# tavildar/Polar

Measured on AMD Instinct MI355X. Metric: codewords/s (N=2048 K=1024 L=32 LLR-SCL), higher is better.
Workload: dtype f64

## Files before the change

polar_amd/build.py:

```python
import os
import shutil
import subprocess
import sys

HERE = os.path.dirname(os.path.abspath(__file__))
ROOT = os.path.dirname(HERE)
CSRC = os.path.join(HERE, "csrc")
INC = os.path.join(ROOT, "include")
LIB = os.path.join(HERE, "libpolar_amd.so")
BUILD = os.path.join(HERE, "_build")
FLAGS_LIST32 = ["-mllvm", "-amdgpu-sched-strategy=max-memory-clause", "-mllvm", "-amdgpu-use-amdgpu-trackers"] + \
               os.environ.get("POLAR_LIST32_FLAGS", "").split()
FLAGS_LAT = os.environ.get("POLAR_LAT_FLAGS", "").split()
SOURCES = [("polar_kernels.hip", ["POLAR_ED_TU=0"], "", []), ("polar_kernels.hip", ["POLAR_ED_TU=1"], ".ed", []),
           ("polar_kernels.hip", ["POLAR_ED_TU=2"], ".ed32", FLAGS_LIST32), ("polar_kernels.hip", ["POLAR_ED_TU=3"], ".lat", FLAGS_LAT),
           ("polar_kernels.hip", ["POLAR_ED_TU=4"], ".list", []),
           ("polar_kernels_sc.hip", [], "", []), ("polar_kernels_p1.hip", [], "", []), ("polar_channel.hip", [], "", []),
           ("polar_construct.hip", [], "", []), ("polar_kernels_mlc.hip", [], "", []), ("polar_kernels_ga.hip", [], "", [])] + \
          [(f, [], "", []) for f in ("polar_handle.cpp", "polar_decode.cpp", "polar_hostpipe.cpp", "polar_montecarlo.cpp", "polar_multi.cpp",
                                     "polar_debug.cpp", "polar_ga.cpp", "polar_bicm.cpp", "polar_list.cpp", "polar_mlc.cpp")]
TEST_HOOK_SOURCES = ("polar_montecarlo.cpp", "polar_debug.cpp")
LIB_TEST = os.path.join(HERE, "libpolar_amd_test.so")
KNOWN_DEFS = {"POLAR_MARGIN", "POLAR_SLOTHIST", "SCLAT_PROF", "POLAR_DEV_GS32", "POLAR_DEV_ONE", "POLAR_NO_FIXED_N",
              "POLAR_NO_GUARD_INT", "POLAR_NO_COLD_HINTS", "OCC", "ED_NR"}
ARCH = os.environ.get("POLAR_ARCH", "gfx950")
_flags_ok = {}


def _probe_flags(flags):
    key = tuple(flags)
    if key not in _flags_ok:
# ... 179 lines not shown
```

polar_amd/csrc/polar_debug.cpp:

```cpp
#include "polar_multi.h"
#include "polar_amd_debug.h"

extern "C" {

int polar_debug_weak_leaves(const polar_code_t *h) { return polar_get_weak_leaves(h); }

int polar_debug_set(polar_code_t *h, const char *key, long value) {
    if (!h || !key) return fail(POLAR_E_ARG, "NULL argument");
    polar_code::Knobs &k = h->knobs;
    const std::string s(key);
    if (s == "mode_override") { if (value < -1 || value > 2) return fail(POLAR_E_ARG, "mode_override must be -1 (none), 0, 1 or 2"); k.mode_override = (int)value; }
    else if (s == "sc_no_fold") k.sc_no_fold = value != 0;
    else if (s == "no_tables") k.no_tables = value != 0;
    else if (s == "no_fuse_front") k.no_fuse_front = value != 0;
    else if (s == "no_prefix") h->prefix_on = (value == 0);
    else if (s == "no_rccl") { k.no_rccl = value != 0; multi_release(h, false); }
    else if (s == "force_rccl") { k.force_rccl = value != 0; multi_release(h, false); }
#ifdef POLAR_TEST_HOOKS
    else if (s == "host_fail_alloc") k.host_fail_alloc = value;
    else if (s == "share_device") { k.share_device = value != 0; multi_release(h, false); }
    else if (s == "fail_device") k.fail_device = (int)value;
    else if (s == "fail_collective") k.fail_collective = (int)value;
#endif
    else if (s == "lat_max_b") k.lat_max_b = value;
    else if (s == "list_chunk_cw") { if (value < 0) return fail(POLAR_E_ARG, "list_chunk_cw must be >= 0"); k.list_chunk_cw = value; }
    else if (s == "host_pipe_min_bytes") k.host_pipe_min_bytes = value;
    else if (s == "host_chunk_bytes") k.host_chunk_bytes = value;
    else if (s == "host_lanes") { if (value < 0 || value > HostPipe::kMaxLanes) return fail(POLAR_E_ARG, "host_lanes must be 0 (default) or 1 .. %d", HostPipe::kMaxLanes); k.host_lanes = value; }
// ... 15 lines not shown
long polar_debug_get(const polar_code_t *h, const char *key) {
    if (!key) return -1;
    const std::string s(key);
    if (s == "allocs") return (long)g_allocs.load();
    if (s == "comm_inits") return (long)polar_debug_comm_inits();
    if (!h) return -1;
    if (s == "test_hooks") {
#ifdef POLAR_TEST_HOOKS
        return 1;
#else
        return 0;
#endif
    }
    if (s == "weak_leaves") return h->weak_leaves;
    if (s == "mode_override") return h->knobs.mode_override;
    if (s == "last_rounds") return h->last_rounds;
    if (s == "last_round_max_per_device") return h->last_round_max_per_device;
    if (s == "worker_threads_started") return h->worker_threads_started;
    if (s.compare(0, 9, "round_us_") == 0) {
        if (h->round_us.empty()) return 0;
        std::vector<long> v(h->round_us);
        if (s == "round_us_count") return (long)v.size();
        if (s == "round_us_first") return v.front();
        std::sort(v.begin(), v.end());
        if (s == "round_us_min") return v.front();
        if (s == "round_us_max") return v.back();
        if (s == "round_us_median") return v[v.size() / 2];
        return -1;
    }
    if (s == "multi_poisoned") return h->multi_poisoned ? 1 : 0;
// ... 14 lines not shown
```

polar_amd/csrc/polar_decode.cpp:

```cpp
#include "polar_host.h"

namespace {

int effective_mode(const polar_code *h) { return h->knobs.mode_override >= 0 ? h->knobs.mode_override : h->mode; }
long lat_resident(const polar_code *h, int gs) {
    const size_t lds = polar_decode_lat_lds_bytes(h->N, gs, h->W);
    return lds <= h->lds_per_block ? (long)h->num_cu * std::min<long>(4, (long)(h->lds_per_block / lds)) : 0;
}
bool use_sc_lat(const polar_code *h, long B) {
    return h->n <= polar_sc_lat_max_log() && polar_sc_lat_lds_bytes(h->N, (int)h->sc_lat_ops.size()) <= h->lds_per_block &&
           h->knobs.lat_max_b >= 0 && B <= (h->knobs.lat_max_b ? h->knobs.lat_max_b : 2048);
}

struct Call {
    polar_code *h;
    const void *d_llr; int llr_fmt; long B; const unsigned int *n_dev; int L; uint8_t *d_out; double *d_pm;
    hipStream_t st; void *ev_start, *ev_stop; int phase; Deferred *deferred;
    BatchGeometry g; PolarDecodeParams p;
};

int batch_setup(polar_code *h, long B, int L, BatchGeometry &g) {
    if (!batch_geometry(h, B, L, true, g)) return fail(POLAR_E_ARG, "lds_log %d does not fit the LDS", g.lds_log);
    if ((size_t)g.grid * g.big * 64 + 64 > h->d_llr_scr.cap) {
        const size_t per_wave = g.big * 64 * sizeof(double) + 1;
// ... 80 lines not shown
    if (int rc = prefix_params(h, g.gs, p)) return rc;
    HIP_TRY(hipMemsetAsync(p.work, 0, sizeof(unsigned int), c.st));
    if (p.prefix_q) HIP_TRY(polar_launch_prefix(p, false, nullptr, c.st));
    if (c.ev_start) HIP_TRY(hipEventRecord((hipEvent_t)c.ev_start, c.st));
    HIP_TRY(polar_launch_decode_llr(p, g.gs, g.lds_log, g.pipe, g.grid, false, c.st));
    if (c.ev_stop) HIP_TRY(hipEventRecord((hipEvent_t)c.ev_stop, c.st));
    return POLAR_OK;
}

int decode_batch_ed(Call &c) {
    polar_code *h = c.h; const BatchGeometry &g = c.g;
    PolarDecodeParams &p = c.p;
    const long B = c.B;
    int rc;
    if ((rc = prefix_params(h, g.gs, p))) return rc;
    HIP_TRY(hipMemsetAsync(p.work, 0, sizeof(unsigned int), c.st));
    if ((rc = h->d_ech.ensure((size_t)B * h->N))) return rc;
    if ((rc = h->d_flags.ensure((size_t)B))) return rc;
    if ((rc = h->d_list.ensure((size_t)B))) return rc;
    if ((rc = h->d_count.ensure(1))) return rc;
    HIP_TRY(hipMemsetAsync(h->d_count.p, 0, sizeof(unsigned int), c.st));
    const bool fuse_front = p.prefix_q > 0 && polar_prefix_is_staged(h->N) && !h->knobs.no_fuse_front;
    if (!fuse_front) HIP_TRY(polar_launch_ed_front(c.d_llr, c.llr_fmt, h->d_ech.p, h->d_flags.p, h->d_tabs.p, h->N, B, c.n_dev, c.st));
    PolarDecodeParams pe = p;
    pe.llr = h->d_ech.p; pe.llr_fmt = POLAR_LLR_F64; pe.flags = h->d_flags.p;
    if (g.gs == 32 && !g.pipe && h->N >= 1024 && p.prefix_q > 0 && !h->knobs.no_tables) {
        if ((rc = h->d_tab_scr.ensure((size_t)g.grid * g.G * 3 * h->N + 64))) return rc;
        if ((rc = h->d_var_scr.ensure((size_t)g.grid * (h->N / 32) * 64 + 64))) return rc;
        pe.tab_scr = h->d_tab_scr.p; pe.var_scr = h->d_var_scr.p;
    }
    if (pe.prefix_q && fuse_front) {
        PolarDecodeParams pp = pe;
        pp.llr = (const double *)c.d_llr; pp.llr_fmt = c.llr_fmt;
        HIP_TRY(polar_launch_prefix(pp, true, h->d_ech.p, c.st));
    } else if (pe.prefix_q) HIP_TRY(polar_launch_prefix(pe, true, nullptr, c.st));
    if (c.ev_start) HIP_TRY(hipEventRecord((hipEvent_t)c.ev_start, c.st));
    HIP_TRY(polar_launch_decode_llr(pe, g.gs, g.lds_log, g.pipe, g.grid, true, c.st));
    if (c.ev_stop) HIP_TRY(hipEventRecord((hipEvent_t)c.ev_stop, c.st));
    HIP_TRY(polar_launch_ed_collect(h->d_flags.p, B, c.n_dev, h->d_list.p, h->d_count.p, c.st));
    return fallback_pass(p, g, h->d_list.p, h->d_count.p, nullptr, h->weak_leaves ? g.grid : 64 * g.wpb, c.st);
}

}

Family polar_host::choose_family(const polar_code *h, long B, int L, bool want_pm) {
    const int mode = effective_mode(h), gs = pow2ceil(L);
    if (L == 1 && mode != 1 && !want_pm) return use_sc_lat(h, B) ? Family::ScLat : Family::Sc8;
    const bool ed = gs >= 4 && mode != 1;
    const long resident = lat_resident(h, gs);
    if ((gs == 2 || (ed && (gs == 4 || gs == 8))) && h->knobs.lat_max_b >= 0 && resident > 0 &&
        B <= (h->knobs.lat_max_b ? h->knobs.lat_max_b : 2 * resident)) return Family::ListLat;
// ... 55 lines not shown
void polar_host::fill_enc(const polar_code *h, PolarEncodeParams &p) {
    memset(&p, 0, sizeof p);
    p.n = h->n; p.N = h->N; p.K = h->K; p.crc = h->crc;
    p.order = h->d_order.p; p.crcm = h->d_crcm.p;
    p.stride = 1;
    p.info_block_div = 100;
}

int polar_host::decode_impl(polar_code *h, const void *d_llr, int llr_fmt, long B, const unsigned int *n_dev, int L, uint8_t *d_out,
                            double *d_pm, void *stream, void *ev_start, void *ev_stop, int phase, Deferred *deferred) {
    if (deferred) *deferred = Deferred::None;
    int rc = check_args(h && d_llr && d_out, L, B);
    if (rc || B == 0) return rc;
    DevGuard dg_;
    if ((rc = ensure_device(h, dg_))) return rc;
    if ((rc = h->d_work.ensure(1))) return rc;
    const Family fam = choose_family(h, B, L, d_pm != nullptr);
    Call c{h, d_llr, llr_fmt, B, n_dev, L, d_out, d_pm, (hipStream_t)stream, ev_start, ev_stop, phase, deferred, {}, {}};
    if (!(fam == Family::ListLat && effective_mode(h) == 1) && (rc = batch_setup(h, B, L, c.g))) return rc;
    base_params(h, L, B, c.p);
    c.p.llr = (const double *)d_llr; c.p.llr_fmt = llr_fmt; c.p.out = d_out; c.p.pm_out = d_pm; c.p.n_dev = n_dev;
    switch (fam) {
        case Family::Sc8: case Family::ScLat: return decode_sc8(c, fam == Family::ScLat);
        case Family::ListLat: return decode_list_lat(c);
        case Family::BatchLlr: return decode_batch_llr(c);
        case Family::BatchEd: break;
    }
    return decode_batch_ed(c);
}

extern "C" {
// ... 127 lines not shown
    int rc = check_args(true, L, B);
    if (rc || B == 0) return rc;
    DevGuard dg_;
    if ((rc = ensure_device(h, dg_))) return rc;
    DevBuf<double> llr, pm;
    DevBuf<uint8_t> out;
    if ((rc = llr.ensure((size_t)B * h->N + 1)) || (rc = out.ensure((size_t)B * h->K)) || (rc = pm.ensure((size_t)B))) { llr.release(); out.release(); pm.release(); return rc; }
    rc = polar_synth_llr_dev(h, 1, 0, B, polar_snr_sqrt_linear(h, 2.0), llr.p, nullptr, nullptr);
    const int top = std::min(pow2ceil(L), POLAR_MAX_LIST);
    for (int l = 1; l <= top && !rc; l <<= 1) {
        rc = polar_decode_scl_llr_batch_dev(h, llr.p, B, l, out.p, nullptr, nullptr);
        if (!rc && l <= 8) rc = polar_decode_scl_llr_batch_dev(h, llr.p, 1, l, out.p, nullptr, nullptr);
        if (!rc && l == 1) rc = polar_decode_scl_llr_batch_dev(h, llr.p, B, l, out.p, pm.p, nullptr);
        if (!rc && l == 1) rc = polar_decode_scl_llr_batch_dev(h, llr.p + 1, B, l, out.p, nullptr, nullptr);
    }
    hipError_t e = hipDeviceSynchronize();
    llr.release(); out.release(); pm.release();
    if (!rc && e != hipSuccess) return fail(POLAR_E_DEVICE, "polar_reserve: %s", hipGetErrorString(e));
    return rc;
}

int polar_count_errors_dev(polar_code_t *h, const uint8_t *d_a, const uint8_t *d_b, long B,
                           unsigned long long *d_err_count, void *stream) {
    int rc = check_args(h && d_a && d_b && d_err_count, kNoList, B);
    if (rc || B == 0) return rc;
    DevGuard dg_;
    if ((rc = ensure_device(h, dg_))) return rc;
    HIP_TRY(polar_launch_count_errors(d_a, d_b, B, h->K, d_err_count, nullptr, (hipStream_t)stream));
    return POLAR_OK;
}
// ... 3 lines not shown
```

polar_amd/csrc/polar_edom.h:

```cpp
#pragma once
#include <hip/hip_runtime.h>
#include <stdint.h>

#include "polar_device.h"

#ifndef POLAR_NO_COLD_HINTS
#define POLAR_UNLIKELY(x) __builtin_expect(!!(x), 0)
#define POLAR_LIKELY(x) __builtin_expect(!!(x), 1)
#else
#define POLAR_UNLIKELY(x) (x)
#define POLAR_LIKELY(x) (x)
#endif
#define POLAR_UNLIKELY2(x) POLAR_UNLIKELY(x)
#define POLAR_LIKELY2(x) POLAR_LIKELY(x)

namespace {

struct Tabs { const double *T, *RC, *LC; };

__device__ __forceinline__ double exp_neg(double x, const Tabs &tb) {
    const double kd = __builtin_rint(x * -92.332482616893657);
    const int k = (int)kd;
    double s = __builtin_fma(kd, -0.010830424696223417, -x);
    s = __builtin_fma(kd, -2.5728046223276688e-14, s);
// ... 52 lines not shown
    const double q = ed_div(fa + fb, __builtin_fma(fa, fb, 1.0));
    const u64 m_hi = __builtin_amdgcn_fcmp(mn, ED_C40_HI, 2);
    const u64 m_lo = __builtin_amdgcn_fcmp(mn, ED_C40_LO, 2);
    const u64 m_l = __builtin_amdgcn_fcmp(mx, 1.0, 2);
    guard |= (m_hi ^ m_lo) & ~m_l;
    double r = __builtin_amdgcn_inverse_ballot_w64(m_hi) ? q : mx;
    if (POLAR_UNLIKELY(m_l != 0)) r = __builtin_amdgcn_inverse_ballot_w64(m_l) ? mn : r;
    return ed_with_sign(r, __double2hiint(a) ^ __double2hiint(b));
}
__device__ __forceinline__ double f_node_e_acc(double a, double b, double &gacc) {
    const double fa = fabs(a), fb = fabs(b);
    const double mx = ed_absmax(a, b), mn = ed_absmin(a, b);
    const double q = ed_div(fa + fb, __builtin_fma(fa, fb, 1.0));
    const u64 m_hi = __builtin_amdgcn_fcmp(mn, ED_C40_HI, 2);
    const u64 m_l = __builtin_amdgcn_fcmp(mx, 1.0, 2);
#if !defined(POLAR_NO_GUARD_INT) && !(defined(POLAR_ED_TU) && POLAR_ED_TU == 2)
    const u64 m_near = __builtin_amdgcn_uicmp((unsigned)__double2hiint(mn), 0x3C539792u, 32);
    double r = __builtin_amdgcn_inverse_ballot_w64(m_hi) ? q : mx;
    if (POLAR_UNLIKELY((m_l | m_near) != 0)) {
        r = __builtin_amdgcn_inverse_ballot_w64(m_l) ? mn : r;
        gacc = ed_absmin(gacc, mn - ED_C40_HI);
    }
#else
    gacc = ed_absmin(gacc, mn - ED_C40_HI);
    double r = __builtin_amdgcn_inverse_ballot_w64(m_hi) ? q : mx;
    if (POLAR_UNLIKELY(m_l != 0)) r = __builtin_amdgcn_inverse_ballot_w64(m_l) ? mn : r;
#endif
    return ed_with_sign(r, __double2hiint(a) ^ __double2hiint(b));
}
constexpr double ED_GACC_FLAG = 4.248354255291589e-18 * 2.0000001e-10;
__device__ __forceinline__ double ed_log(double x, const Tabs &tb) {
// ... 46 lines not shown
```

polar_amd/csrc/polar_handle.cpp:

```cpp
#include "polar_host.h"

namespace polar_host {

thread_local std::string g_err;

int fail(int code, const char *fmt, ...) {
    char buf[512];
    va_list ap;
    va_start(ap, fmt);
    vsnprintf(buf, sizeof buf, fmt, ap);
    va_end(ap);
    g_err = buf;
    return code;
}

std::atomic<unsigned long> g_allocs{0};

int usable_cpus() {
    int n = (int)std::thread::hardware_concurrency();
    cpu_set_t set;
    if (sched_getaffinity(0, sizeof set, &set) == 0) n = CPU_COUNT(&set);
    if (FILE *f = fopen("/sys/fs/cgroup/cpu.max", "r")) {
        char q[32]; long per = 0;
        if (fscanf(f, "%31s %ld", q, &per) == 2 && strcmp(q, "max") != 0 && per > 0) n = std::min<long>(n, std::max<long>(1, atol(q) / per));
// ... 179 lines not shown
        }
        if ((rc = upload(h->d_tabs, t))) return rc;
    }
    h->dev_ready = true;
    return POLAR_OK;
}

int read_env_knobs(polar_code *h) {
    auto on = [](const char *name) { const char *e = getenv(name); return e && *e && strcmp(e, "0") != 0; };
    if (const char *e = getenv("POLAR_MODE")) {
        if (!(e[0] >= '0' && e[0] <= '2' && e[1] == 0)) return fail(POLAR_E_ARG, "POLAR_MODE=%s: must be 0, 1 or 2", e);
        h->knobs.mode_override = e[0] - '0';
    }
    h->knobs.sc_no_fold = on("POLAR_SC_NO_FOLD");
    h->knobs.no_tables = on("POLAR_NO_TABLES");
    h->knobs.no_rccl = on("POLAR_NO_RCCL");
    h->knobs.force_rccl = on("POLAR_FORCE_RCCL");
    return POLAR_OK;
}

void drop_clones(polar_code *h) {
    if (h->multi_poisoned) return;
    for (polar_code *c : h->clones) polar_destroy(c);
    h->clones.clear();
    if (h->hpipe) for (polar_code *&c : h->hpipe->ctx) if (c) { polar_destroy(c); c = nullptr; }
}

}

extern "C" {
// ... 71 lines not shown
    {
        int cur = -1;
        if (h->dev_ready && hipGetDevice(&cur) == hipSuccess && cur != h->device) dg_.prev = cur;
    }
    if (h->dev_ready) (void)hipSetDevice(h->device);
    h->d_frozen.release(); h->d_ctl.release(); h->d_crcm.release(); h->d_order.release(); h->d_info_rank.release();
    h->d_crc_mask.release(); h->d_tabs.release(); h->d_pre.release(); h->d_llr_scr.release(); h->d_c_scr.release(); h->d_hist_scr.release();
    h->d_in.release(); h->d_f32.release(); h->d_out.release(); h->d_bytes_a.release(); h->d_bytes_b.release();
    h->d_counter.release(); h->d_sel.release(); h->d_work.release();
    h->d_ech.release(); h->d_flags.release(); h->d_list.release(); h->d_count.release(); h->d_bicm_llr.release(); h->d_list_out.release();
    h->d_alive[0].release(); h->d_alive[1].release(); h->d_nalive.release(); h->d_mc_ctr.release();
    for (auto &sl : h->mc_slots) { sl.list[0].release(); sl.list[1].release(); }
    h->d_slot_n.release();
    if (h->pin_in) (void)hipHostFree(h->pin_in);
    if (h->pin_out) (void)hipHostFree(h->pin_out);
    h->d_sc_ops.release(); h->d_sc_lat_ops.release(); h->d_flag_words.release(); h->d_var_scr.release(); h->d_tab_scr.release();
    delete h;
}

int polar_get_params(const polar_code_t *h, int *n, int *N, int *K, int *crc) {
    if (!h) return fail(POLAR_E_ARG, "NULL handle");
    if (n) *n = h->n;
    if (N) *N = h->N;
    if (K) *K = h->K;
    if (crc) *crc = h->crc;
    return POLAR_OK;
}
int polar_get_frozen(const polar_code_t *h, uint8_t *o) {
    if (!h || !o) return fail(POLAR_E_ARG, "NULL argument");
    memcpy(o, h->frozen.data(), h->N); return POLAR_OK;
}
// ... 55 lines not shown
```

polar_amd/csrc/polar_host.h:

```cpp
#pragma once
#include <hip/hip_runtime.h>

#include <dlfcn.h>
#include <sched.h>
#include <sys/mman.h>
#include <unistd.h>

#include <algorithm>
#include <atomic>
#include <chrono>
#include <condition_variable>
#include <memory>
#include <mutex>
#include <thread>
#include <cmath>
#include <cstdarg>
#include <cstdio>
#include <cstdlib>
#include <cstring>
#include <functional>
#include <numeric>
#include <string>
#include <vector>

// ... 174 lines not shown
    std::vector<uint16_t> info_rank;
    std::vector<uint32_t> crc_mask;
    std::vector<uint8_t> sched;
    std::vector<uint32_t> ctl;
    int weak_leaves = 0;
    std::vector<uint32_t> sc_ops;
    std::vector<uint32_t> sc_lat_ops;
    bool sc_fold = false;
    bool dev_ready = false;
    int device = -1, num_cu = 0;
    size_t lds_per_block = 0;
    DevBuf<uint8_t> d_frozen, d_crcm;
    DevBuf<uint16_t> d_order, d_info_rank;
    DevBuf<uint32_t> d_crc_mask, d_ctl, d_sc_ops, d_sc_lat_ops, d_var_scr;
    DevBuf<double> d_tab_scr;
    DevBuf<unsigned int> d_flag_words;
    DevBuf<double> d_llr_scr, d_tabs, d_pre;
    DevBuf<uint32_t> d_c_scr, d_hist_scr;
    DevBuf<double> d_in;
    DevBuf<float> d_f32;
    DevBuf<uint8_t> d_out, d_bytes_a, d_bytes_b;
    DevBuf<unsigned long long> d_counter;
    DevBuf<unsigned int> d_work;
    DevBuf<uint64_t> d_sel;
    DevBuf<double> d_ech;
    DevBuf<uint8_t> d_flags;
    DevBuf<uint32_t> d_list;
    DevBuf<unsigned int> d_count;
    DevBuf<double> d_list_out;
    DevBuf<double> d_bicm_llr;
    int mode = 0;
    struct Knobs {
        int mode_override = -1;
        bool sc_no_fold = false;
        bool no_tables = false;
        bool no_fuse_front = false;
        bool no_rccl = false;
        bool force_rccl = false;
        bool share_device = false;
        int fail_device = -1;
        int fail_collective = -1;
        long multi_timeout_s = 1800;
        long multi_grace_s = 10;
        bool force_workers = false;
        int stall_device = -1;
        long stall_ms = 0;
        long lat_max_b = 0;
        long host_pipe_min_bytes = 0;
        long host_chunk_bytes = 0;
        long host_lanes = 0;
// ... 104 lines not shown
```

polar_amd/csrc/polar_kernels.h:

```cpp
#pragma once
#include <hip/hip_runtime.h>
#include <stdint.h>
#include <stddef.h>

#ifndef POLAR_LLR_F64
#define POLAR_LLR_F64  0
#define POLAR_LLR_F32  1
#define POLAR_LLR_F16  2
#define POLAR_LLR_BF16 3
#endif
static inline size_t polar_llr_esz(int fmt) { return fmt == POLAR_LLR_F64 ? 8 : fmt == POLAR_LLR_F32 ? 4 : 2; }

struct PolarDecodeParams {
    int n, N, K, crc, L;
    int W;
    int prefix_q, prefix_len;
    long B;
    const double *llr;
    int llr_fmt;
    const double *p0;
    uint8_t *out;
    double *pm_out;
    const uint8_t *frozen;
    const uint32_t *ctl;
// ... 8 lines not shown
    uint8_t *flags;
    const uint32_t *cw_list;
    const unsigned int *cw_count;
    const unsigned int *n_dev;
    double *tab_scr;
    uint32_t *var_scr;
};
struct PolarListParams : PolarDecodeParams {
    uint8_t *list_cand;
    double *list_pm;
    uint8_t *list_crc;
    int32_t *list_nact;
    int32_t *list_win;
};

static inline int polar_decode_waves_per_block(int pipe) { return pipe ? 1 : 4; }
static inline size_t polar_decode_lds_bytes(int lds_log, int pipe) {
    return 324 * 8 + (size_t)polar_decode_waves_per_block(pipe) * ((size_t)((2u << lds_log) - 1) * 64 * 8 + 128 * 8 + 128);
}
static inline size_t polar_decode_big(int N, int lds_log) { return N > (2 << lds_log) ? (size_t)(N - (2 << lds_log)) : 0; }
static inline size_t polar_decode_cwords(int N) { return N >= 128 ? (size_t)(N / 32 - 2) : 0; }
hipError_t polar_launch_prefix(const PolarDecodeParams &p, bool ed, double *ech_out, hipStream_t st);
hipError_t polar_launch_prefix_ed0(const PolarDecodeParams &p, double *ech_out, hipStream_t st);
hipError_t polar_launch_prefix_ed1(const PolarDecodeParams &p, double *ech_out, hipStream_t st);
int polar_prefix_is_staged(int N);
hipError_t polar_launch_decode_llr_ed0(const PolarDecodeParams &p, int gs, int lds_log, int pipe, int grid, hipStream_t st);
hipError_t polar_launch_decode_llr_ed1(const PolarDecodeParams &p, int gs, int lds_log, int pipe, int grid, hipStream_t st);
hipError_t polar_launch_decode_lat(const PolarDecodeParams &p, int gs, bool ed, int blocks, hipStream_t st);
size_t polar_decode_lat_lds_bytes(int N, int gs, int W);
hipError_t polar_launch_decode_llr(const PolarDecodeParams &p, int gs, int lds_log, int pipe, int grid, bool ed, hipStream_t st);
// ... 174 lines not shown
```

polar_amd/csrc/polar_kernels.hip:

```cpp
#include <hip/hip_runtime.h>
#include <stdint.h>
#include <type_traits>

#include "polar_kernels.h"
#include "polar_device.h"
#include "polar_edom.h"

#ifdef POLAR_PROFILE
#define PROF_DECL u64 prof_acc[24] = {0,0,0,0,0,0,0,0,0,0,0,0,0,0,0,0,0,0,0,0,0,0,0,0}; u64 prof_t = __builtin_readcyclecounter();
#define PROF(i) { u64 t_ = __builtin_readcyclecounter(); prof_acc[i] += t_ - prof_t; prof_t = t_; }
#define PROF_OUT if (lane == 0 && p.pm_out) { for (int i_ = 0; i_ < 24; ++i_) atomicAdd((u64 *)p.pm_out + i_, prof_acc[i_]); }
#define PROF_CNT(i, v) { prof_acc[i] += (u64)(v); }
#else
#define PROF_DECL
#define PROF(i)
#define PROF_CNT(i, v)
#define PROF_OUT
#endif

#include "polar_llr_nodes.h"

template <bool NARROW16>
__device__ __forceinline__ const double *ch_row(const PolarDecodeParams &p, size_t cw, int N) {
    if constexpr (NARROW16) {
        if (p.llr_fmt >= POLAR_LLR_F16) return reinterpret_cast<const double *>(reinterpret_cast<const uint16_t *>(p.llr) + cw * (size_t)N);
    }
    return p.llr_fmt ? reinterpret_cast<const double *>(reinterpret_cast<const float *>(p.llr) + cw * (size_t)N)
                     : p.llr + cw * (size_t)N;
// ... 12 lines not shown
#define POLAR_SKIP_L1 1
#endif
#define POLAR_SADDR 1
#ifndef OCC
#define OCC 4
#endif
#define LANE_CTX                                   \
    const int lane = LAT ? lane_k : lane_id_opaque();    \
    const int lig = lane & (GS - 1);               \
    const int gbase = lane & ~(GS - 1);            \
    (void)lig; (void)gbase;
#if defined(POLAR_ED_TU) && POLAR_ED_TU == 4
#define POLAR_LIST_OUT 1
#define scl_decode_llr_kernel scl_decode_llr_list_kernel
#define POLAR_KPARAMS PolarListParams
#else
#define POLAR_KPARAMS PolarDecodeParams
#endif
template <int GS, int LDS_LOG, int PIPE, bool ED, int NL = 0, int LAT = 0>
__global__ __launch_bounds__(PIPE ? 64 : 256, PIPE ? 2 : OCC) void scl_decode_llr_kernel(POLAR_KPARAMS p) {
    constexpr int WPB = PIPE ? 1 : 4;
    constexpr bool CH_N16 = !ED;
    constexpr int G = LAT ? 1 : 64 / GS;
    constexpr int EL = 64 / GS;
    constexpr int CST = LAT ? GS : 64;
#define POLAR_CL (LAT ? lig : lane)
#define POLAR_CGB (LAT ? 0 : gbase)
    constexpr int SL = 1 << LDS_LOG;
    const int lane = threadIdx.x & 63;
    const int wib = __builtin_amdgcn_readfirstlane((int)(threadIdx.x >> 6));
    const int wave_id = blockIdx.x * WPB + wib;
    const int nwaves = gridDim.x * WPB;
// ... 79 lines not shown
                    x[k] = (i < N) ? (p.llr_fmt ? llr_load_narrow(p.llr, row + i, p.llr_fmt) : p.llr[row + i]) : 1.0;
                }
#pragma unroll
                for (int k = 0; k < 8; ++k) {
                    const int i = i0 + 64 * k + lane;
                    double v = x[k];
                    if constexpr (ED) { bool f; v = ed_from_channel(x[k], tb, f); any |= f; sized |= fabs(x[k]) >= 0.1; }
                    if (i < N) lat_ch[__brev((unsigned)i) >> (32 - n)] = v;
                }
            }
            if constexpr (ED) { if (wave_any(any) || !wave_any(sized)) guard = ~0ull; }
        }
        wave_mem_fence();

        int phi_start = 0, forced_top = 0;
        const double *pre_cw = nullptr;
        if (!LAT && p.prefix_q > 0) {
            const int Q = p.prefix_q, Pe = p.prefix_len;
            pre_cw = p.pre + (size_t)(valid ? cw : 0) * (size_t)(N - Q + 1);
            if (active) {
                pm = pre_cw[0];
                for (int S = 64; S <= Q && S <= N / 2; S <<= 1) {
                    uint32_t *cz = g_cl + (size_t)(S / 32 - 2) * 64 + lane;
                    for (int w = 0; w < S / 32; ++w) cz[(size_t)w * 64] = 0u;
                    pC.set(__builtin_ctz((unsigned)S), lig);
                }
            }
            wave_mem_fence();
            phi_start = Pe;
            if (Pe < Q) forced_top = n - __builtin_ctz((unsigned)Q) + 1;
        }

        PROF_DECL
#ifdef POLAR_MARGIN
        double mingap = __builtin_inf();
#endif
        typedef const uint32_t __attribute__((address_space(4))) *kconst_u32;
        const kconst_u32 ctlp = (kconst_u32)(uintptr_t)p.ctl;
        uint32_t ctlv = 0, ctlv_n = 0;
        double lat_x[4] = {0.0, 0.0, 0.0, 0.0}, lat_y0 = 0.0, lat_y1 = 0.0;
        bool lat_yv = false;
        (void)lat_x; (void)lat_y0; (void)lat_y1; (void)lat_yv;
        auto ctl_window = [&](int w0) -> uint32_t { const int i_ = w0 + lane_id_opaque(); return p.ctl[i_ < N ? i_ : 0]; };
        uint32_t ctl_next;
        if constexpr (LAT) {
            ctlv = ctl_window(phi_start & ~63);
            ctlv_n = ctl_window((phi_start & ~63) + 64);
            ctl_next = (uint32_t)__builtin_amdgcn_readlane((int)ctlv, phi_start & 63);
        } else ctl_next = ctlp[phi_start];
        for (int phi = phi_start; phi < N; ++phi) {
            PROF(0)
            const uint32_t ctl = ctl_next;
            auto update_c = [&](int S, uint32_t X, int ph) {
                LANE_CTX
                if constexpr (LAT) {
                    if (S == 1 && N >= 128) {
                        uint32_t lo = (uint32_t)clsmall, hi = (uint32_t)(clsmall >> 32);
                        bool done = false;
                        auto level = [&](auto SC_) {
                            constexpr int Sc = decltype(SC_)::value;
                            if (done) return;
                            const uint32_t cl = (Sc == 16) ? (lo >> 16) : ((lo >> Sc) & ((1u << Sc) - 1u));
                            const uint32_t nw = (cl ^ X) | (X << Sc);
                            if (!((ph >> 1) & 1)) {
                                if constexpr (Sc == 16) hi = nw;
// ... 58 lines not shown
                    ph = psi;
                }
            };
            const int zb = (int)(ctl >> 1) & 0x7F;
            {
                const int nphi = phi + (1 << zb);
                if constexpr (LAT) {
                    if (POLAR_UNLIKELY2(((nphi ^ phi) & ~63) != 0)) { ctlv = ctlv_n; ctlv_n = ctl_window((nphi & ~63) + 64); }
                    ctl_next = (uint32_t)__builtin_amdgcn_readlane((int)ctlv, nphi & 63);
                } else ctl_next = ctlp[nphi < N ? nphi : 0];
            }
            const int lam_stop = n - zb;
#include "polar_scl_visits.inc"
#include "polar_scl_leaf.inc"
        }
        PROF_OUT

#include "polar_scl_finish.inc"
        if (p.work) {
            unsigned nxt = 0;
            if (lane == 0) nxt = atomicAdd(p.work, 1u);
            g0 = ((long)nwaves + (long)__builtin_amdgcn_readfirstlane((int)nxt)) * G;
        } else {
            g0 += (long)nwaves * G;
        }
    }
}

template <bool ED>
__global__ __launch_bounds__(256) void prefix_kernel(PolarDecodeParams p, int staged, double *ech_out) {
    __shared__ double tabs[324];
    extern __shared__ double pstage[];

// ... 319 lines not shown
    return hipGetLastError();
}
hipError_t polar_launch_decode_llr_list(const PolarListParams &p, int gs, int grid, hipStream_t st) {
    if (!p.list_cand || grid < 4 || (grid & 3)) return hipErrorInvalidValue;
    switch (gs) {
        case 1: return launch_list<1>(p, grid, st);
        case 2: return launch_list<2>(p, grid, st);
        case 4: return launch_list<4>(p, grid, st);
        case 8: return launch_list<8>(p, grid, st);
        case 16: return launch_list<16>(p, grid, st);
        case 32: return launch_list<32>(p, grid, st);
        case 64: return launch_list<64>(p, grid, st);
        default: return hipErrorInvalidValue;
    }
}
#elif POLAR_ED_TU == 2
hipError_t polar_launch_decode_llr_ed1_gs32(const PolarDecodeParams &p, int lds_log, int pipe, int grid, hipStream_t st) {
    return launch_gs<32, true>(p, lds_log, pipe, grid, st);
}
#elif POLAR_ED_TU == 1
hipError_t polar_launch_decode_llr_ed1_gs32(const PolarDecodeParams &p, int lds_log, int pipe, int grid, hipStream_t st);
hipError_t polar_launch_decode_llr_ed1(const PolarDecodeParams &p, int gs, int lds_log, int pipe, int grid, hipStream_t st) {
    switch (gs) {
#ifndef POLAR_DEV_GS32
        case 4: return launch_gs<4, true>(p, lds_log, pipe, grid, st);
        case 8: return launch_gs<8, true>(p, lds_log, pipe, grid, st);
        case 16: return launch_gs<16, true>(p, lds_log, pipe, grid, st);
        case 64: return launch_gs<64, true>(p, lds_log, pipe, grid, st);
#endif
        case 32: return polar_launch_decode_llr_ed1_gs32(p, lds_log, pipe, grid, st);
// ... 23 lines not shown
```

polar_amd/csrc/polar_scl_visits.inc:

```
            const int lam_top = (phi == phi_start && forced_top) ? forced_top : (phi ? (n - __builtin_ctz((unsigned)phi)) : 1);
            double leaf = 0.0;
            if constexpr (LAT) {
                const bool bottom_regs = n >= 3;
                const int lam_hi = bottom_regs ? (lam_stop < n - 2 ? lam_stop : n - 2) : lam_stop;
                for (int lam = lam_top; lam <= lam_hi; ++lam) {
                    const int sh_ = n - lam, S_ = 1 << sh_, e_ = lane_k / GS;
                    const bool odd_ = (phi >> sh_) & 1;
                    const int pin_ = (lam > 1) ? pL.get(sh_ + 1) : 0;
                    const double *srcp = (lam > 1) ? lat_a + (size_t)(2 * S_ - 1) * GS + pin_ : lat_ch;
                    const int sstr = (lam > 1) ? GS : 1;
                    double *dstp = lat_a + (size_t)(S_ - 1) * GS + lig;
                    const uint32_t *cwp_ = (odd_ && S_ > 32) ? g_cl + (size_t)(S_ / 32 - 2) * CST + pC.get(sh_) : nullptr;
                    auto one = [&](int j, double a_, double b_) -> double {
                        if (!odd_) return FN(a_, b_);
                        if (S_ <= 32) return GN(a_, b_, (uint32_t)(clsmall >> S_), j);
                        return GN(a_, b_, cwp_[(size_t)(j >> 5) * CST], j & 31);
                    };
                    if (S_ == 1) {
                        if (!(odd_ && lat_yv)) { lat_y0 = srcp[0]; lat_y1 = srcp[sstr]; }
                        lat_yv = !odd_;
                        leaf = one(0, lat_y0, lat_y1);
                        PROF(4)
                        continue;
                    }
// ... 177 lines not shown
                                    double x0, x1;
                                    if (odd) {
                                        const int bi = (S > 32) ? ((j + k) & 31) : (j + k);
                                        x0 = GN(a0[k], b0[k], cb0, bi);
                                        x1 = GN(a1[k], b1[k], cb1, bi);
                                    } else {
                                        x0 = FN(a0[k], b0[k]);
                                        x1 = FN(a1[k], b1[k]);
                                    }
                                    out0[(size_t)(j + k) * 64] = x0;
                                    out0[(size_t)(j + k + H) * 64] = x1;
                                    out1[(size_t)(j + k) * 64] = FN(x0, x1);
                                }
                            }
                        };
                        const bool tsrc = tbl && lam == 3 && phi >= S2;
                        auto fused4 = [&](const double *inp, double *o0, double *o1, double *o2, double *o3, auto NTT, auto TSS, auto GMM) {
                            constexpr bool TS = decltype(TSS)::value;
                            constexpr int GM = decltype(GMM)::value;
                            const uint32_t lb = (uint32_t)lane * 8u;
                            const uint32_t lin = (uint32_t)(gbase + pin) * 8u;
                            const char *inu = reinterpret_cast<const char *>(g_llr + (size_t)(2 * S - 2 * SL) * 64);
                            auto st = [&](double *o, auto gbit, auto ntbit, size_t row, double val) {
                                constexpr bool G_ = decltype(gbit)::value, N_ = decltype(ntbit)::value;
                                double *q_ = G_ ? reinterpret_cast<double *>(reinterpret_cast<char *>(o) + row * 512 + lb) : o + row * 64;
                                if (N_) __builtin_nontemporal_store(val, q_); else *q_ = val;
                            };
                            constexpr int NT = decltype(NTT)::value;
                            const int E = S >> 3;
                            uint32_t cw8[8] = {0, 0, 0, 0, 0, 0, 0, 0};
                            if (odd && S <= 32) cw8[0] = (uint32_t)(clsmall >> S);
// ... 263 lines not shown
```

Before: 1.023 million.

## Split list-32 decode into narrow head phase and state-importing tail phase

```diff
diff --git a/polar_amd/build.py b/polar_amd/build.py
--- a/polar_amd/build.py
+++ b/polar_amd/build.py
@@ -15,6 +15,7 @@
 SOURCES = [("polar_kernels.hip", ["POLAR_ED_TU=0"], "", []), ("polar_kernels.hip", ["POLAR_ED_TU=1"], ".ed", []),
            ("polar_kernels.hip", ["POLAR_ED_TU=2"], ".ed32", FLAGS_LIST32), ("polar_kernels.hip", ["POLAR_ED_TU=3"], ".lat", FLAGS_LAT),
            ("polar_kernels.hip", ["POLAR_ED_TU=4"], ".list", []),
+           ("polar_kernels.hip", ["POLAR_ED_TU=5"], ".headA", []), ("polar_kernels.hip", ["POLAR_ED_TU=6"], ".headB", FLAGS_LIST32),
            ("polar_kernels_sc.hip", [], "", []), ("polar_kernels_p1.hip", [], "", []), ("polar_channel.hip", [], "", []),
            ("polar_construct.hip", [], "", []), ("polar_kernels_mlc.hip", [], "", []), ("polar_kernels_ga.hip", [], "", [])] + \
           [(f, [], "", []) for f in ("polar_handle.cpp", "polar_decode.cpp", "polar_hostpipe.cpp", "polar_montecarlo.cpp", "polar_multi.cpp",
diff --git a/polar_amd/csrc/polar_debug.cpp b/polar_amd/csrc/polar_debug.cpp
--- a/polar_amd/csrc/polar_debug.cpp
+++ b/polar_amd/csrc/polar_debug.cpp
@@ -1,5 +1,8 @@
 #include "polar_multi.h"
 #include "polar_amd_debug.h"
+#ifdef POLAR_TEST_HOOKS
+#include "polar_head_plan.h"
+#endif
 
 extern "C" {
 
@@ -12,6 +15,8 @@
     if (s == "mode_override") { if (value < -1 || value > 2) return fail(POLAR_E_ARG, "mode_override must be -1 (none), 0, 1 or 2"); k.mode_override = (int)value; }
     else if (s == "sc_no_fold") k.sc_no_fold = value != 0;
     else if (s == "no_tables") k.no_tables = value != 0;
+    else if (s == "no_head") k.no_head = value != 0;
+    else if (s == "head_min_b") { if (value < 0) return fail(POLAR_E_ARG, "head_min_b must be >= 0 (0 = default)"); k.head_min_b = value; }
     else if (s == "no_fuse_front") k.no_fuse_front = value != 0;
     else if (s == "no_prefix") h->prefix_on = (value == 0);
     else if (s == "no_rccl") { k.no_rccl = value != 0; multi_release(h, false); }
@@ -57,6 +62,27 @@
     }
     if (s == "weak_leaves") return h->weak_leaves;
     if (s == "mode_override") return h->knobs.mode_override;
+    if (s == "head_phi") return h->last_head_phi;
+#ifdef POLAR_TEST_HOOKS
+    if (s == "head_check") {
+        if (!h->last_head_phi || h->last_head_b <= 0 || !h->d_head_rec.p) return -2;
+        int P = 0;
+        while (P < h->N && h->frozen[P]) ++P;
+        const int Q = P >= 256 ? 256 : (P < 33 ? 0 : (P < 64 ? 64 : (P < 128 ? 128 : 256)));
+        const HeadPlan hp = head_plan(h->frozen.data(), h->n, Q, std::min(P, Q), h->N / 2);
+        if (hp.phi_h != h->last_head_phi) return -3;
+        std::vector<unsigned long long> rows2((size_t)h->last_head_b * 4);
+        const size_t pitch = hp.record_words() * sizeof(unsigned long long);
+        if (hipMemcpy2D(rows2.data(), 32, h->d_head_rec.p + 2 * 4, pitch, 32, (size_t)h->last_head_b, hipMemcpyDeviceToHost) != hipSuccess) return -4;
+        long bad = 0;
+        for (long b = 0; b < h->last_head_b; ++b) {
+            unsigned long long r[4];
+            for (int a = 0; a < 4; ++a) r[a] = rows2[(size_t)b * 4 + a];
+            bad += head_record_ok(hp, r) ? 0 : 1;
+        }
+        return bad;
+    }
+#endif
     if (s == "last_rounds") return h->last_rounds;
     if (s == "last_round_max_per_device") return h->last_round_max_per_device;
     if (s == "worker_threads_started") return h->worker_threads_started;
diff --git a/polar_amd/csrc/polar_decode.cpp b/polar_amd/csrc/polar_decode.cpp
--- a/polar_amd/csrc/polar_decode.cpp
+++ b/polar_amd/csrc/polar_decode.cpp
@@ -1,4 +1,5 @@
 #include "polar_host.h"
+#include "polar_head_plan.h"
 
 namespace {
 
@@ -118,7 +119,7 @@
     const long B = c.B;
     int rc;
     if ((rc = prefix_params(h, g.gs, p))) return rc;
-    HIP_TRY(hipMemsetAsync(p.work, 0, sizeof(unsigned int), c.st));
+    HIP_TRY(hipMemsetAsync(p.work, 0, 2 * sizeof(unsigned int), c.st));
     if ((rc = h->d_ech.ensure((size_t)B * h->N))) return rc;
     if ((rc = h->d_flags.ensure((size_t)B))) return rc;
     if ((rc = h->d_list.ensure((size_t)B))) return rc;
@@ -138,7 +139,28 @@
         pp.llr = (const double *)c.d_llr; pp.llr_fmt = c.llr_fmt;
         HIP_TRY(polar_launch_prefix(pp, true, h->d_ech.p, c.st));
     } else if (pe.prefix_q) HIP_TRY(polar_launch_prefix(pe, true, nullptr, c.st));
+    HeadPlan hp;
+    if (g.gs == 32 && p.prefix_q > 0) hp = head_plan(h->frozen.data(), h->n, p.prefix_q, p.prefix_len, h->N / 2);
+    const long head_min_b = h->knobs.head_min_b ? h->knobs.head_min_b : (long)h->num_cu * 16 * 16;
+    const bool two_phase = head_use(hp, g.lds_log == 3 && !g.pipe, B, head_min_b, h->knobs.no_head);
+    h->last_head_phi = two_phase ? hp.phi_h : 0;
+    h->last_head_b = two_phase && !c.n_dev ? B : 0;
+    PolarHeadParams ph;
+    if (two_phase) {
+        if ((rc = h->d_head_rec.ensure((size_t)B * hp.record_words()))) return rc;
+        static_cast<PolarDecodeParams &>(ph) = pe;
+        ph.head_rec = h->d_head_rec.p; ph.head_phi = hp.phi_h; ph.head_t = hp.t; ph.head_rows = hp.rows();
+        ph.head_llr_mask = hp.llr_mask; ph.head_c_mask = hp.c_mask;
+    }
     if (c.ev_start) HIP_TRY(hipEventRecord((hipEvent_t)c.ev_start, c.st));
+    if (two_phase) {
+        PolarHeadParams pa = ph;
+        pa.L = HeadPlan::kPaths; pa.work = p.work + 1; pa.tab_scr = nullptr; pa.var_scr = nullptr; pa.out = nullptr; pa.pm_out = nullptr;
+        const long waves_a = (B + 15) / 16;
+        const int grid_a = (int)std::min<long>(g.grid, ((waves_a + g.wpb - 1) / g.wpb) * g.wpb);
+        HIP_TRY(polar_launch_decode_head_export(pa, grid_a, c.st));
+        HIP_TRY(polar_launch_decode_head_import(ph, g.grid, c.st));
+    } else
     HIP_TRY(polar_launch_decode_llr(pe, g.gs, g.lds_log, g.pipe, g.grid, true, c.st));
     if (c.ev_stop) HIP_TRY(hipEventRecord((hipEvent_t)c.ev_stop, c.st));
     HIP_TRY(polar_launch_ed_collect(h->d_flags.p, B, c.n_dev, h->d_list.p, h->d_count.p, c.st));
@@ -224,7 +246,8 @@
     if (rc || B == 0) return rc;
     DevGuard dg_;
     if ((rc = ensure_device(h, dg_))) return rc;
-    if ((rc = h->d_work.ensure(1))) return rc;
+    if ((rc = h->d_work.ensure(2))) return rc;
+    h->last_head_phi = 0; h->last_head_b = 0;
     const Family fam = choose_family(h, B, L, d_pm != nullptr);
     Call c{h, d_llr, llr_fmt, B, n_dev, L, d_out, d_pm, (hipStream_t)stream, ev_start, ev_stop, phase, deferred, {}, {}};
     if (!(fam == Family::ListLat && effective_mode(h) == 1) && (rc = batch_setup(h, B, L, c.g))) return rc;
@@ -382,6 +405,14 @@
         if (!rc && l == 1) rc = polar_decode_scl_llr_batch_dev(h, llr.p, B, l, out.p, pm.p, nullptr);
         if (!rc && l == 1) rc = polar_decode_scl_llr_batch_dev(h, llr.p + 1, B, l, out.p, nullptr, nullptr);
     }
+    if (!rc && top >= 32) {
+        PolarDecodeParams pp;
+        base_params(h, 32, B, pp);
+        if (!(rc = prefix_params(h, 32, pp)) && pp.prefix_q > 0) {
+            const HeadPlan hp = head_plan(h->frozen.data(), h->n, pp.prefix_q, pp.prefix_len, h->N / 2);
+            if (hp.phi_h > 0 && hp.window >= kHeadMinWindow) rc = h->d_head_rec.ensure((size_t)B * hp.record_words());
+        }
+    }
     hipError_t e = hipDeviceSynchronize();
     llr.release(); out.release(); pm.release();
     if (!rc && e != hipSuccess) return fail(POLAR_E_DEVICE, "polar_reserve: %s", hipGetErrorString(e));
diff --git a/polar_amd/csrc/polar_edom.h b/polar_amd/csrc/polar_edom.h
--- a/polar_amd/csrc/polar_edom.h
+++ b/polar_amd/csrc/polar_edom.h
@@ -90,7 +90,7 @@
     const double q = ed_div(fa + fb, __builtin_fma(fa, fb, 1.0));
     const u64 m_hi = __builtin_amdgcn_fcmp(mn, ED_C40_HI, 2);
     const u64 m_l = __builtin_amdgcn_fcmp(mx, 1.0, 2);
-#if !defined(POLAR_NO_GUARD_INT) && !(defined(POLAR_ED_TU) && POLAR_ED_TU == 2)
+#if !defined(POLAR_NO_GUARD_INT) && !(defined(POLAR_ED_TU) && (POLAR_ED_TU == 2 || POLAR_ED_TU == 6))
     const u64 m_near = __builtin_amdgcn_uicmp((unsigned)__double2hiint(mn), 0x3C539792u, 32);
     double r = __builtin_amdgcn_inverse_ballot_w64(m_hi) ? q : mx;
     if (POLAR_UNLIKELY((m_l | m_near) != 0)) {
diff --git a/polar_amd/csrc/polar_handle.cpp b/polar_amd/csrc/polar_handle.cpp
--- a/polar_amd/csrc/polar_handle.cpp
+++ b/polar_amd/csrc/polar_handle.cpp
@@ -217,6 +217,7 @@
     }
     h->knobs.sc_no_fold = on("POLAR_SC_NO_FOLD");
     h->knobs.no_tables = on("POLAR_NO_TABLES");
+    h->knobs.no_head = on("POLAR_NO_HEAD");
     h->knobs.no_rccl = on("POLAR_NO_RCCL");
     h->knobs.force_rccl = on("POLAR_FORCE_RCCL");
     return POLAR_OK;
@@ -318,7 +319,7 @@
     h->d_slot_n.release();
     if (h->pin_in) (void)hipHostFree(h->pin_in);
     if (h->pin_out) (void)hipHostFree(h->pin_out);
-    h->d_sc_ops.release(); h->d_sc_lat_ops.release(); h->d_flag_words.release(); h->d_var_scr.release(); h->d_tab_scr.release();
+    h->d_sc_ops.release(); h->d_sc_lat_ops.release(); h->d_flag_words.release(); h->d_var_scr.release(); h->d_tab_scr.release(); h->d_head_rec.release();
     delete h;
 }
 
diff --git a/polar_amd/csrc/polar_head_plan.h b/polar_amd/csrc/polar_head_plan.h
--- /dev/null
+++ b/polar_amd/csrc/polar_head_plan.h
@@ -0,0 +1,53 @@
+#pragma once
+#include <cstddef>
+#include <cstdint>
+#include <vector>
+
+struct HeadPlan {
+    int phi_h = 0;
+    int paths = 0;
+    int t = 0;
+    int window = 0;
+    uint32_t llr_mask = 0;
+    uint32_t c_mask = 0;
+    int llr_rows = 0, c_rows = 0;
+    static constexpr int kFixedRows = 3, kPaths = 4;
+    int rows() const { return kFixedRows + c_rows + llr_rows; }
+    size_t record_words() const { return (size_t)rows() * kPaths; }
+};
+
+inline HeadPlan head_plan(const uint8_t *frozen, int n, int Q, int Pe, int phi_cap) {
+    HeadPlan hp;
+    const int N = 1 << n;
+    if (Q <= 0 || N < 64) return hp;
+    int unf[3], k = 0;
+    for (int i = 0; i < N && k < 3; ++i) if (!frozen[i]) unf[k++] = i;
+    if (k < 3) return hp;
+    int phi = unf[2] & ~15;
+    if (phi >= phi_cap) phi = (phi_cap - 1) & ~15;
+    if (phi <= Pe || phi <= 0) return hp;
+    hp.phi_h = phi;
+    hp.t = (unf[0] < phi) + (unf[1] < phi);
+    hp.paths = 1 << hp.t;
+    hp.window = phi - Pe;
+    for (int s = 5; s < n; ++s) {
+        const int T = 1 << s, m = phi & (T - 1);
+        if (m > 0 && m <= T / 2 && !(T >= Q && phi < T)) { hp.llr_mask |= 1u << s; hp.llr_rows += T; }
+    }
+    for (int s = 6; s < n; ++s)
+        if (phi & (1 << s)) { hp.c_mask |= 1u << s; hp.c_rows += (1 << s) / 32; }
+    return hp;
+}
+
+constexpr int kHeadMinWindow = 64;
+inline bool head_use(const HeadPlan &hp, bool default_tuning, long B, long min_b, bool disabled) {
+    return !disabled && default_tuning && hp.phi_h > 0 && B >= min_b && hp.window >= kHeadMinWindow;
+}
+
+inline bool head_record_ok(const HeadPlan &hp, const unsigned long long (&row2)[HeadPlan::kPaths]) {
+    for (int a = 0; a < HeadPlan::kPaths; ++a) {
+        if ((int)((row2[a] >> 32) & 0x7FFFFFFFull) != hp.t) return false;
+        if (((row2[a] >> 63) != 0) != (a >= HeadPlan::kPaths - hp.paths)) return false;
+    }
+    return true;
+}
diff --git a/polar_amd/csrc/polar_host.h b/polar_amd/csrc/polar_host.h
--- a/polar_amd/csrc/polar_host.h
+++ b/polar_amd/csrc/polar_host.h
@@ -212,6 +212,9 @@
     DevBuf<uint16_t> d_order, d_info_rank;
     DevBuf<uint32_t> d_crc_mask, d_ctl, d_sc_ops, d_sc_lat_ops, d_var_scr;
     DevBuf<double> d_tab_scr;
+    DevBuf<unsigned long long> d_head_rec;
+    int last_head_phi = 0;
+    long last_head_b = 0;
     DevBuf<unsigned int> d_flag_words;
     DevBuf<double> d_llr_scr, d_tabs, d_pre;
     DevBuf<uint32_t> d_c_scr, d_hist_scr;
@@ -232,6 +235,8 @@
         int mode_override = -1;
         bool sc_no_fold = false;
         bool no_tables = false;
+        bool no_head = false;
+        long head_min_b = 0;
         bool no_fuse_front = false;
         bool no_rccl = false;
         bool force_rccl = false;
diff --git a/polar_amd/csrc/polar_kernels.h b/polar_amd/csrc/polar_kernels.h
--- a/polar_amd/csrc/polar_kernels.h
+++ b/polar_amd/csrc/polar_kernels.h
@@ -46,6 +46,14 @@
     int32_t *list_win;
 };
 
+struct PolarHeadParams : PolarDecodeParams {
+    unsigned long long *head_rec;
+    int head_phi, head_t, head_rows;
+    uint32_t head_llr_mask, head_c_mask;
+};
+hipError_t polar_launch_decode_head_export(const PolarHeadParams &p, int grid, hipStream_t st);
+hipError_t polar_launch_decode_head_import(const PolarHeadParams &p, int grid, hipStream_t st);
+
 static inline int polar_decode_waves_per_block(int pipe) { return pipe ? 1 : 4; }
 static inline size_t polar_decode_lds_bytes(int lds_log, int pipe) {
     return 324 * 8 + (size_t)polar_decode_waves_per_block(pipe) * ((size_t)((2u << lds_log) - 1) * 64 * 8 + 128 * 8 + 128);
diff --git a/polar_amd/csrc/polar_kernels.hip b/polar_amd/csrc/polar_kernels.hip
--- a/polar_amd/csrc/polar_kernels.hip
+++ b/polar_amd/csrc/polar_kernels.hip
@@ -11,7 +11,13 @@
 #define PROF(i) { u64 t_ = __builtin_readcyclecounter(); prof_acc[i] += t_ - prof_t; prof_t = t_; }
 #define PROF_OUT if (lane == 0 && p.pm_out) { for (int i_ = 0; i_ < 24; ++i_) atomicAdd((u64 *)p.pm_out + i_, prof_acc[i_]); }
 #define PROF_CNT(i, v) { prof_acc[i] += (u64)(v); }
+#define PROF_HEAD_DECL const int prof_head_phi = p.pm_out ? (int)((const u64 *)p.pm_out)[32] : 0; const u64 prof_head_t0 = prof_t; bool prof_head_open = prof_head_phi > 0;
+#define PROF_HEAD(phi_) if (prof_head_open && (phi_) >= prof_head_phi) { prof_acc[22] += __builtin_readcyclecounter() - prof_head_t0; prof_head_open = false; }
+#define PROF_HEAD_END prof_acc[23] += __builtin_readcyclecounter() - prof_head_t0;
 #else
+#define PROF_HEAD_DECL
+#define PROF_HEAD(phi_)
+#define PROF_HEAD_END
 #define PROF_DECL
 #define PROF(i)
 #define PROF_CNT(i, v)
@@ -54,8 +60,15 @@
 #define POLAR_LIST_OUT 1
 #define scl_decode_llr_kernel scl_decode_llr_list_kernel
 #define POLAR_KPARAMS PolarListParams
+#elif defined(POLAR_ED_TU) && (POLAR_ED_TU == 5 || POLAR_ED_TU == 6)
+#define POLAR_HEAD (POLAR_ED_TU == 5 ? 1 : 2)
+#define scl_decode_llr_kernel scl_decode_llr_head_kernel
+#define POLAR_KPARAMS PolarHeadParams
 #else
 #define POLAR_KPARAMS PolarDecodeParams
+#endif
+#ifndef POLAR_HEAD
+#define POLAR_HEAD 0
 #endif
 template <int GS, int LDS_LOG, int PIPE, bool ED, int NL = 0, int LAT = 0>
 __global__ __launch_bounds__(PIPE ? 64 : 256, PIPE ? 2 : OCC) void scl_decode_llr_kernel(POLAR_KPARAMS p) {
@@ -165,6 +178,54 @@
         wave_mem_fence();
 
         int phi_start = 0, forced_top = 0;
+#if POLAR_HEAD == 2
+        {
+            static_assert(GS == 32 && ED && !LAT && !PIPE && LDS_LOG == 3, "import exists for the list of 32 in its default tuning");
+            const int la = lig - (L - 4);
+            const bool mine = valid && la >= 0 && lig < L;
+            const u64 *rec = p.head_rec + (size_t)(valid ? cw : 0) * (size_t)p.head_rows * 4 + (mine ? la : 0);
+            const u64 st_ = mine ? rec[8] : 0ull;
+            active = (st_ >> 63) != 0;
+            actw = __ballot(active);
+            sp = L - __popcll((actw >> gbase) & gmask);
+            if (active) {
+                pm = __longlong_as_double((long long)rec[0]);
+                clsmall = rec[4];
+                hword = (uint32_t)st_;
+                int r = 3;
+                for (int s = 6; s < n; ++s) {
+                    if (!((p.head_c_mask >> s) & 1u)) continue;
+                    const int nwd = (1 << s) / 32;
+                    uint32_t *dst = g_cl + (size_t)(nwd - 2) * 64 + lane;
+#pragma unroll 1
+                    for (int w = 0; w < nwd; w += 2) {
+                        const u64 x0 = rec[(size_t)(r + w) * 4], x1 = rec[(size_t)(r + w + 1) * 4];
+                        dst[(size_t)w * 64] = (uint32_t)x0; dst[(size_t)(w + 1) * 64] = (uint32_t)x1;
+                    }
+                    pC.set(s, lig);
+                    r += nwd;
+                }
+                for (int s = 5; s < n; ++s) {
+                    if (!((p.head_llr_mask >> s) & 1u)) continue;
+                    const int T = 1 << s;
+                    double *dst = g_llr + (size_t)(T - 2 * SL) * 64 + lane;
+#pragma unroll 1
+                    for (int j = 0; j < T; j += 4) {
+                        u64 x[4];
+#pragma unroll
+                        for (int k = 0; k < 4; ++k) x[k] = rec[(size_t)(r + j + k) * 4];
+#pragma unroll
+                        for (int k = 0; k < 4; ++k) dst[(size_t)(j + k) * 64] = __longlong_as_double((long long)x[k]);
+                    }
+                    pL.set(s, lig);
+                    r += T;
+                }
+            }
+            t = (unsigned)p.head_t;
+            wave_mem_fence();
+            phi_start = p.head_phi;
+        }
+#else
         const double *pre_cw = nullptr;
         if (!LAT && p.prefix_q > 0) {
             const int Q = p.prefix_q, Pe = p.prefix_len;
@@ -181,8 +242,10 @@
             phi_start = Pe;
             if (Pe < Q) forced_top = n - __builtin_ctz((unsigned)Q) + 1;
         }
+#endif
 
         PROF_DECL
+        PROF_HEAD_DECL
 #ifdef POLAR_MARGIN
         double mingap = __builtin_inf();
 #endif
@@ -199,7 +262,12 @@
             ctlv_n = ctl_window((phi_start & ~63) + 64);
             ctl_next = (uint32_t)__builtin_amdgcn_readlane((int)ctlv, phi_start & 63);
         } else ctl_next = ctlp[phi_start];
+#if POLAR_HEAD == 1
+        for (int phi = phi_start; phi < p.head_phi; ++phi) {
+#else
         for (int phi = phi_start; phi < N; ++phi) {
+#endif
+            PROF_HEAD(phi)
             PROF(0)
             const uint32_t ctl = ctl_next;
             auto update_c = [&](int S, uint32_t X, int ph) {
@@ -288,9 +356,52 @@
 #include "polar_scl_visits.inc"
 #include "polar_scl_leaf.inc"
         }
+        PROF_HEAD_END
         PROF_OUT
 
+#if POLAR_HEAD == 1
+        {
+            static_assert(GS == 4 && ED && !LAT && !PIPE && LDS_LOG == 3, "export exists for the groups of 4 lanes in the default tuning");
+            (void)K; (void)g_tb;
+            if (valid) {
+                u64 *rec = p.head_rec + (size_t)cw * (size_t)p.head_rows * 4 + lig;
+                rec[0] = active ? (u64)__double_as_longlong(pm) : 0ull;
+                rec[4] = clsmall;
+                rec[8] = (u64)hword | ((u64)t << 32) | ((u64)(active ? 1 : 0) << 63);
+                if (active) {
+                    int r = 3;
+                    for (int s = 6; s < n; ++s) {
+                        if (!((p.head_c_mask >> s) & 1u)) continue;
+                        const int nwd = (1 << s) / 32;
+                        const uint32_t *src = g_cl + (size_t)(nwd - 2) * 64 + gbase + pC.get(s);
+                        for (int w = 0; w < nwd; w += 2) {
+                            const uint32_t x0 = src[(size_t)w * 64], x1 = src[(size_t)(w + 1) * 64];
+                            rec[(size_t)(r + w) * 4] = x0; rec[(size_t)(r + w + 1) * 4] = x1;
+                        }
+                        r += nwd;
+                    }
+                    for (int s = 5; s < n; ++s) {
+                        if (!((p.head_llr_mask >> s) & 1u)) continue;
+                        const int T = 1 << s;
+                        const double *src = g_llr + (size_t)(T - 2 * SL) * 64 + gbase + pL.get(s);
+                        for (int j = 0; j < T; j += 8) {
+                            double x[8];
+#pragma unroll
+                            for (int k = 0; k < 8; ++k) x[k] = src[(size_t)(j + k) * 64];
+#pragma unroll
+                            for (int k = 0; k < 8; ++k) rec[(size_t)(r + j + k) * 4] = (u64)__double_as_longlong(x[k]);
+                        }
+                        r += T;
+                    }
+                }
+            }
+            guard |= __ballot(gacc <= ED_GACC_FLAG);
+            if (valid && lig == 0 && ((guard >> gbase) & gmask) != 0) p.flags[cw] = 1;
+            wave_mem_fence();
+        }
+#else
 #include "polar_scl_finish.inc"
+#endif
         if (p.work) {
             unsigned nxt = 0;
             if (lane == 0) nxt = atomicAdd(p.work, 1u);
@@ -640,6 +751,24 @@
         default: return hipErrorInvalidValue;
     }
 }
+#elif POLAR_ED_TU == 5
+hipError_t polar_launch_decode_head_export(const PolarHeadParams &p, int grid, hipStream_t st) {
+    if (!p.head_rec || p.L != 4 || p.head_phi <= 0 || p.head_phi >= p.N || grid < 4 || (grid & 3)) return hipErrorInvalidValue;
+    hipLaunchKernelGGL((scl_decode_llr_kernel<4, 3, 0, true>), dim3(grid / 4), dim3(256), polar_decode_lds_bytes(3, 0), st, p);
+    return hipGetLastError();
+}
+#elif POLAR_ED_TU == 6
+hipError_t polar_launch_decode_head_import(const PolarHeadParams &p, int grid, hipStream_t st) {
+    if (!p.head_rec || p.L < 17 || p.L > 32 || p.head_phi <= 0 || p.head_phi >= p.N || grid < 4 || (grid & 3)) return hipErrorInvalidValue;
+    const size_t lds = polar_decode_lds_bytes(3, 0);
+#ifndef POLAR_NO_FIXED_N
+    if (p.n == 11) hipLaunchKernelGGL((scl_decode_llr_kernel<32, 3, 0, true, 11>), dim3(grid / 4), dim3(256), lds, st, p);
+    else if (p.n == 10) hipLaunchKernelGGL((scl_decode_llr_kernel<32, 3, 0, true, 10>), dim3(grid / 4), dim3(256), lds, st, p);
+    else
+#endif
+    hipLaunchKernelGGL((scl_decode_llr_kernel<32, 3, 0, true>), dim3(grid / 4), dim3(256), lds, st, p);
+    return hipGetLastError();
+}
 #elif POLAR_ED_TU == 2
 hipError_t polar_launch_decode_llr_ed1_gs32(const PolarDecodeParams &p, int lds_log, int pipe, int grid, hipStream_t st) {
     return launch_gs<32, true>(p, lds_log, pipe, grid, st);
diff --git a/polar_amd/csrc/polar_scl_visits.inc b/polar_amd/csrc/polar_scl_visits.inc
--- a/polar_amd/csrc/polar_scl_visits.inc
+++ b/polar_amd/csrc/polar_scl_visits.inc
@@ -215,7 +215,11 @@
                                 }
                             }
                         };
+#if POLAR_HEAD == 2
+                        const bool tsrc = tbl && lam == 3 && phi >= S2 && (phi >= S1 || p.head_phi <= S2);
+#else
                         const bool tsrc = tbl && lam == 3 && phi >= S2;
+#endif
                         auto fused4 = [&](const double *inp, double *o0, double *o1, double *o2, double *o3, auto NTT, auto TSS, auto GMM) {
                             constexpr bool TS = decltype(TSS)::value;
                             constexpr int GM = decltype(GMM)::value;
```

After: 1.062 million, median of 6. +3.8%, better.
